# jeremy-collins/sd-video-gen

Hardware: AMD Instinct MI355X
Metric: generated frames/sec at 50 DDIM denoise steps, 512x512 (higher is better)
Workload: dtype fp16; 1 GPU; configs[2]: 1_16_kitti_L1_64 F=64, 64x64 latents -> 512x512 VAE passes, 50-step DDIM; --denoise --denoise_start_step 0, guidance_scale 0; SD-v1.4 UNet at 64x64 latents, VAE enc/dec at 512x512; clips_per_gpu=56, streams_per_gpu=2, pred_frames=1, global_clips=56, parallelism=clip-sharded dp1, weights=seeded random init (SD v1.4 architecture, 1_16_kitti_L1_64)

## Files before the change

sd-video-gen_amd/csrc/ff_fused.hip:

```cpp
#include "igemm_epi.h"
#include <vector>

namespace SDNS {

namespace {

constexpr int FC = 320;
constexpr int FH = 1280;
constexpr int F_SLAB = 16384;
#ifndef FF_DEPTH
#define FF_DEPTH 4
#endif
constexpr int F_DEPTH = FF_DEPTH;
constexpr int F_KS = FC / 32;
constexpr int F_NCH = FH / 64;
constexpr int F_SPC = 5 + 3;

struct FfArgs {
  const h16* X; int ldx;
  const h16* W1; const float* b1; const float* s1;
  const float* rs; const float* rm;
  const h16* W2p; const float* b2;
  const h16* residual; int ldr;
  h16* out; int ldo;
  int M;
};

constexpr int P_RING = 7;
constexpr int P_OFF_S1 = P_RING * F_SLAB;
constexpr int P_OFF_EX = P_OFF_S1 + 2 * 2 * FH * 4;
constexpr int P_LDS = P_OFF_EX + 8 * 2 * 64 * 16;

#ifdef FF_STAMP
#define FSTAMP(v) do { __builtin_amdgcn_sched_barrier(0); asm volatile("s_memtime %0\n\ts_waitcnt lgkmcnt(0)" : "=s"(v) :: "memory"); __builtin_amdgcn_sched_barrier(0); } while (0)
#else
#define FSTAMP(v) do { } while (0)
#endif

__global__ void __launch_bounds__(512, 2) ff_pair_kernel(const FfArgs a, unsigned long long* stamps) {
  extern __shared__ __attribute__((aligned(16))) char smem[];
  const int tid = threadIdx.x, lane = tid & 63, wid = tid >> 6;
  const int wave_u = __builtin_amdgcn_readfirstlane(wid);
  const int pair_u = wave_u >> 1, half_u = wave_u & 1;
  const int l15 = lane & 15, lq = lane >> 4;
  const int m0 = blockIdx.x * 128;
  const unsigned lds0 = (unsigned)(uintptr_t)((__attribute__((address_space(3))) char*)smem);
  constexpr unsigned INVALID = 0x80000000u;

  const uint64_t p1 = (uint64_t)a.W1, p2 = (uint64_t)a.W2p;
  const v4i srd1 = {(int)(unsigned)p1, (int)((p1 >> 32) & 0xffff), (int)(2u * FH * FC * 2u), 0x00020000};
  const v4i srd2 = {(int)(unsigned)p2, (int)((p2 >> 32) & 0xffff), (int)((unsigned)FC * FH * 2u), 0x00020000};

  const int prow = lane >> 3;
  auto dma_slab = [&](int q, int slot) {
    const int c = q >> 3, s = q & 7;
    const unsigned dst = lds0 + slot * F_SLAB;
#pragma unroll
    for (int i = 0; i < 2; ++i) {
      const int blk = i * 8 + wave_u;
      const int row = blk * 8 + prow;
      const int ch = (lane & 7) ^ (row & 7);
      if (s < 5) {
        const unsigned voff = (unsigned)((128 * c + row) * FC + ch * 8) * 2u;
        dma16(srd1, voff, s * 128, dst + blk * 1024);
      } else {
        const int rr = 64 * (s - 5) + (row & 63);
        const int cperm = 32 * (rr >> 5) + 8 * ((rr & 15) >> 2) + 4 * ((rr >> 4) & 1) + (rr & 3);
        const int r = (row >> 6) * 160 + cperm;
        const unsigned voff = rr < 160 ? (unsigned)(r * FH + ch * 8) * 2u : INVALID;
        dma16(srd2, voff, c * 128, dst + blk * 1024);
      }
    }
  };
  constexpr int NQ = F_NCH * F_SPC;
#pragma unroll
  for (int q = 0; q < F_DEPTH; ++q) dma_slab(q, q);

  {
    float* ss = (float*)(smem + P_OFF_S1);
    for (int i = tid; i < 2 * FH; i += 512) { ss[i] = a.s1[i]; ss[2 * FH + i] = a.b1[i]; }
    asm volatile("s_waitcnt lgkmcnt(0)" ::: "memory");
  }
  int mrow[2]; bool m_ok[2];
  h16x8 xf[2][F_KS];
#pragma unroll
  for (int rt = 0; rt < 2; ++rt) {
    mrow[rt] = m0 + pair_u * 32 + rt * 16 + l15;
    m_ok[rt] = mrow[rt] < a.M;
#pragma unroll
    for (int ks = 0; ks < F_KS; ++ks) {
      uint4 v = make_uint4(0, 0, 0, 0);
      if (m_ok[rt]) v = *(const uint4*)(a.X + (int64_t)mrow[rt] * a.ldx + ks * 32 + lq * 8);
      xf[rt][ks] = *(h16x8*)&v;
    }
  }
  float rs[2], rm[2];
#pragma unroll
  for (int rt = 0; rt < 2; ++rt) {
    if (a.rs) {
      rs[rt] = m_ok[rt] ? a.rs[mrow[rt]] : 0.f; rm[rt] = m_ok[rt] ? a.rm[mrow[rt]] : 0.f;
    } else {
      float sum = 0.f;
#pragma unroll
      for (int ks = 0; ks < F_KS; ++ks)
#pragma unroll
        for (int j = 0; j < 8; ++j) sum += (float)xf[rt][ks][j];
      sum += __shfl_xor(sum, 16); sum += __shfl_xor(sum, 32);
      const float mean = sum * (1.f / FC);
      float sq = 0.f;
#pragma unroll
      for (int ks = 0; ks < F_KS; ++ks)
#pragma unroll
        for (int j = 0; j < 8; ++j) { const float dlt = (float)xf[rt][ks][j] - mean; sq += dlt * dlt; }
      sq += __shfl_xor(sq, 16); sq += __shfl_xor(sq, 32);
      rs[rt] = m_ok[rt] ? rsqrtf(sq * (1.f / FC) + 1e-5f) : 0.f;
      rm[rt] = rs[rt] * mean;
    }
  }

  f32x4 acc2[2][10];
#pragma unroll
  for (int rt = 0; rt < 2; ++rt)
#pragma unroll
    for (int t = 0; t < 10; ++t) acc2[rt][t] = f32x4{0.f, 0.f, 0.f, 0.f};

  int fsw[2];
#pragma unroll
  for (int kk = 0; kk < 2; ++kk) fsw[kk] = (half_u * 64 + l15) * 128 + (((kk * 4 + lq) ^ (l15 & 7)) << 4);
  const float* const sS1 = (const float*)(smem + P_OFF_S1);
  const float* const sB1 = sS1 + 2 * FH;
  char* const ex_own = smem + P_OFF_EX + ((wave_u * 2) * 64 + lane) * 16;
  const char* const ex_other = smem + P_OFF_EX + (((wave_u ^ 1) * 2) * 64 + lane) * 16;

  int q = 0, slot = 0, slot_in = F_DEPTH;
  unsigned long long t_wait = 0, t_bar = 0, t_dma = 0, t_g1 = 0, t_gelu = 0, t_g2 = 0, t_all0 = 0, t_all1 = 0, t_epi = 0;
  auto step_sync = [&]() {
    unsigned long long u0 = 0, u1 = 0, u2 = 0;
    FSTAMP(u0);
    if (q + F_DEPTH - 1 < NQ) asm volatile("s_waitcnt vmcnt(6)" ::: "memory");
    else wait_vm((NQ - 1 - q) * 2);
    FSTAMP(u1);
    bar();
    FSTAMP(u2);
    t_wait += u1 - u0; t_bar += u2 - u1;
  };
  auto step_dma = [&]() {
    unsigned long long u2 = 0, u3 = 0;
    FSTAMP(u2);
    if (q + F_DEPTH < NQ) dma_slab(q + F_DEPTH, slot_in);
    FSTAMP(u3);
    t_dma += u3 - u2;
    slot_in = slot_in + 1 == P_RING ? 0 : slot_in + 1;
  };
  auto step_end = [&]() { ++q; slot = slot + 1 == P_RING ? 0 : slot + 1; };
#ifndef FF_STAGGER
#define FF_STAGGER 1
#endif
  const bool late = FF_STAGGER && wave_u >= 4;

  FSTAMP(t_all0);
  for (int c = 0; c < F_NCH; ++c) {
    f32x4 acc1[2][4];
#pragma unroll
    for (int rt = 0; rt < 2; ++rt)
#pragma unroll
      for (int t = 0; t < 4; ++t) acc1[rt][t] = f32x4{0.f, 0.f, 0.f, 0.f};
    h16x8 wpend[4];
    auto rd1 = [&](const char* sl, int kk, h16x8 (&wf)[4]) {
#pragma unroll
      for (int t = 0; t < 4; ++t) wf[t] = *(const h16x8*)(sl + t * 2048 + fsw[kk]);
    };
    auto mm1 = [&](int ks, const h16x8 (&wf)[4]) {
#pragma unroll
      for (int t = 0; t < 4; ++t)
#pragma unroll
        for (int rt = 0; rt < 2; ++rt) acc1[rt][t] = MFMA_16x16x32(wf[t], xf[rt][ks], acc1[rt][t]);
    };
#pragma unroll
    for (int s = 0; s < 5; ++s) {
      step_sync();
      unsigned long long v0 = 0, v1 = 0;
      FSTAMP(v0);
      const char* sl = smem + slot * F_SLAB;
      if (late && s > 0) mm1((s - 1) * 2 + 1, wpend);
      step_dma();
      {
        h16x8 wf[4];
        rd1(sl, 0, wf);
        mm1(s * 2, wf);
      }
      rd1(sl, 1, wpend);
      if (!late || s == 4) mm1(s * 2 + 1, wpend);
#ifdef FF_STAMP
#pragma unroll
      for (int rt = 0; rt < 2; ++rt)
#pragma unroll
        for (int t = 0; t < 4; ++t) asm volatile("" : "+v"(acc1[rt][t]));
#endif
      FSTAMP(v1);
      t_g1 += v1 - v0;
      step_end();
    }
    unsigned long long w0 = 0, w1 = 0;
    FSTAMP(w0);
    h16x8 pown[2];
#pragma unroll
    for (int rt = 0; rt < 2; ++rt) {
#pragma unroll
      for (int pr = 0; pr < 2; ++pr) {
        const int n = 128 * c + 64 * half_u + 32 * pr + 4 * lq;
        const f32x4 sh = *(const f32x4*)(sS1 + n), sg = *(const f32x4*)(sS1 + n + 16);
        const f32x4 bh = *(const f32x4*)(sB1 + n), bg = *(const f32x4*)(sB1 + n + 16);
        const f32x4 h = acc1[rt][2 * pr] * rs[rt] - sh * rm[rt] + bh;
        const f32x4 gt = acc1[rt][2 * pr + 1] * rs[rt] - sg * rm[rt] + bg;
        const f32x4 pv = h * gelu_erf4(gt);
#pragma unroll
        for (int e = 0; e < 4; ++e) pown[rt][pr * 4 + e] = (h16)pv[e];
      }
      *(h16x8*)(ex_own + rt * 1024) = pown[rt];
    }
    asm volatile("s_waitcnt lgkmcnt(0)" ::: "memory");
    FSTAMP(w1);
    t_gelu += w1 - w0;
    h16x8 pf[2][2];
    auto rd2 = [&](const char* sl, int kk, h16x8 (&wf)[4]) {
#pragma unroll
      for (int t = 0; t < 4; ++t) wf[t] = *(const h16x8*)(sl + t * 2048 + fsw[kk]);
    };
    auto mm2 = [&](int s, int kk, const h16x8 (&wf)[4]) {
#pragma unroll
      for (int t = 0; t < 4; ++t) {
        if (s * 4 + t < 10) {
#pragma unroll
          for (int rt = 0; rt < 2; ++rt) acc2[rt][s * 4 + t] = MFMA_16x16x32(wf[t], pf[rt][kk], acc2[rt][s * 4 + t]);
        }
      }
    };
#pragma unroll
    for (int s = 0; s < 3; ++s) {
      step_sync();
      unsigned long long v0 = 0, v1 = 0;
      FSTAMP(v0);
      if (s == 0) {
#pragma unroll
        for (int rt = 0; rt < 2; ++rt) {
          const h16x8 po = *(const h16x8*)(ex_other + rt * 1024);
          pf[rt][0] = half_u ? po : pown[rt];
          pf[rt][1] = half_u ? pown[rt] : po;
        }
      }
      const char* sl = smem + slot * F_SLAB;
      if (late && s > 0) mm2(s - 1, 1, wpend);
      step_dma();
      {
        h16x8 wf[4];
        rd2(sl, 0, wf);
        mm2(s, 0, wf);
      }
      rd2(sl, 1, wpend);
      if (!late || s == 2) mm2(s, 1, wpend);
#ifdef FF_STAMP
#pragma unroll
      for (int rt = 0; rt < 2; ++rt)
#pragma unroll
        for (int t = 0; t < 4; ++t) if (s * 4 + t < 10) asm volatile("" : "+v"(acc2[rt][s * 4 + t]));
#endif
      FSTAMP(v1);
      t_g2 += v1 - v0;
      step_end();
    }
  }
  FSTAMP(t_all1);

#pragma unroll
  for (int rt = 0; rt < 2; ++rt) {
    if (!m_ok[rt]) continue;
    const int m = mrow[rt];
#pragma unroll
    for (int p = 0; p < 5; ++p) {
      const int n = half_u * 160 + 32 * p + 8 * lq;
      f32x4 v0 = acc2[rt][2 * p] + *(const f32x4*)(a.b2 + n);
      f32x4 v1 = acc2[rt][2 * p + 1] + *(const f32x4*)(a.b2 + n + 4);
      if (a.residual) {
        const h16x8 r = *(const h16x8*)(a.residual + (int64_t)m * a.ldr + n);
#pragma unroll
        for (int e = 0; e < 4; ++e) { v0[e] += (float)r[e]; v1[e] += (float)r[4 + e]; }
      }
      h16x8 w;
      const h16x4 w0 = to_h16x4(v0), w1 = to_h16x4(v1);
#pragma unroll
      for (int e = 0; e < 4; ++e) { w[e] = w0[e]; w[4 + e] = w1[e]; }
      *(h16x8*)(a.out + (int64_t)m * a.ldo + n) = w;
    }
  }
#ifdef FF_STAMP
  FSTAMP(t_epi);
  if (stamps && lane == 0) {
    unsigned long long* o = stamps + ((size_t)blockIdx.x * 8 + wid) * 8;
    o[0] = t_wait; o[1] = t_bar; o[2] = t_dma; o[3] = t_g1; o[4] = t_gelu; o[5] = t_g2; o[6] = t_all1 - t_all0; o[7] = t_epi - t_all1;
  }
#endif
}

__global__ void pack_ff2_perm_kernel(const float* __restrict__ w, h16* __restrict__ out, int N, int K) {
  const int64_t total = (int64_t)N * K;
  for (int64_t idx = (int64_t)blockIdx.x * blockDim.x + threadIdx.x; idx < total; idx += (int64_t)gridDim.x * blockDim.x) {
    const int n = (int)(idx / K), k = (int)(idx - (int64_t)n * K);
    const int b = k >> 5, p = k & 31, lq = p >> 3, j = p & 7;
    out[idx] = (h16)w[(int64_t)n * K + 32 * b + 16 * (j >> 2) + 4 * lq + (j & 3)];
  }
}

}

void ff_fused_init_device() {
  HIP_OK(hipFuncSetAttribute((const void*)ff_pair_kernel, hipFuncAttributeMaxDynamicSharedMemorySize, P_LDS));
}

bool ff_fused_supported(int C, int M) {
  return C == FC && M >= 128 * 192;
}

void pack_ff2_perm(const float* w, h16* out, int N, int K, hipStream_t s) {
  const int64_t total = (int64_t)N * K;
  hipLaunchKernelGGL(pack_ff2_perm_kernel, dim3((unsigned)std::min<int64_t>((total + 255) / 256, 4096)), dim3(256), 0, s, w, out, N, K);
  check_launch("pack_ff2_perm");
}

void ff_fused(svg_ctx* ctx, const h16* X, int ldx, const h16* W1, const float* b1, const float* s1,
              const h16* W2p, const float* b2, const h16* residual, int ldr, h16* out, int ldo, int M, hipStream_t s) {
  SVG_CHECK(ldx % 8 == 0 && ldr % 8 == 0 && ldo % 8 == 0 && (int64_t)M * ldx < (1LL << 31), "ff_fused: strides / size unsupported");
  if (!SVG_LAUNCHING(ctx)) return;
  char tag[64];
  snprintf(tag, sizeof(tag), "ff_fused_M%d_C%d", M, FC);
  ProfScope ps(ctx, PK_GEMM, s, 2.0 * M * (double)FC * (2 * FH) + 2.0 * M * (double)FH * FC,
               2.0 * ((double)M * FC * 3 + 3.0 * FC * FH), tag);
  FfArgs a{X, ldx, W1, b1, s1, nullptr, nullptr, W2p, b2, residual, ldr, out, ldo, M};
  unsigned long long* stamps = nullptr;
#ifdef FF_STAMP
  const size_t n_st = (size_t)cdiv(M, 128) * 64;
  HIP_OK(hipMalloc(&stamps, n_st * sizeof(unsigned long long)));
  HIP_OK(hipMemsetAsync(stamps, 0, n_st * sizeof(unsigned long long), s));
#endif
  hipLaunchKernelGGL(ff_pair_kernel, dim3(cdiv(M, 128)), dim3(512), P_LDS, s, a, stamps);
  check_launch("ff_fused");
#ifdef FF_STAMP
  {
    HIP_OK(hipStreamSynchronize(s));
    std::vector<unsigned long long> h(n_st);
    HIP_OK(hipMemcpy(h.data(), stamps, n_st * sizeof(unsigned long long), hipMemcpyDeviceToHost));
    HIP_OK(hipFree(stamps));
    double sum[8] = {0};
    for (size_t w = 0; w < n_st / 8; ++w) for (int k = 0; k < 8; ++k) sum[k] += (double)h[w * 8 + k];
    const double nw = (double)(n_st / 8);
    fprintf(stderr, "[ff stamps] M %d: per wave (cycles, 160 slab steps): ring wait %.0f | barrier %.0f | DMA issue %.0f | GEMM1 slabs (100 x: 8 reads + 16 MFMA) %.0f | "
            "LN-fold + GEGLU + swap write (20 x) %.0f | GEMM2 slabs (60 x: reads + up to 16 MFMA) %.0f || main loop %.0f, epilogue %.0f; matrix time of the loop = 2400 MFMA x 16 = 38400\n",
            M, sum[0] / nw, sum[1] / nw, sum[2] / nw, sum[3] / nw, sum[4] / nw, sum[5] / nw, sum[6] / nw, sum[7] / nw);
  }
#endif
}

}
```

sd-video-gen_amd/csrc/xattn_fused.hip:

```cpp
#include "igemm_epi.h"
#include <cstdlib>

namespace SDNS {

namespace {

constexpr int XC = 320, XH = 8, XD = 40, XDP = 48;
constexpr int XQ = XH * XDP;
constexpr int X_SLAB = 16384;
constexpr int X_RING = 8, X_DEPTH = 4;
constexpr int X_KS = XC / 32;
constexpr int X_P0 = 15, X_P1 = 15, X_P2 = 2 * XH, X_P3 = 18;
constexpr int X_OFF_C = X_RING * X_SLAB;
constexpr int X_LDS = X_OFF_C + (2 * XQ + XC) * 4;
constexpr int X_HEAD_ELEMS = 128 * 64;

struct XaArgs {
  const h16* X; int ldx;
  const h16* R; int ldr;
  const h16* Wp; const float* bp;
  const float* rs; const float* rm;
  const h16* Wq; const float* sq; const float* bq;
  const h16* Kp; const h16* Vp;
  const h16* Wo; const float* bo;
  h16* out; int ldo;
  int M, rows_per_sample, L;
  float scale_log2e;
};

__device__ __forceinline__ h16x8 cat8(h16x4 a, h16x4 b) { return __builtin_shufflevector(a, b, 0, 1, 2, 3, 4, 5, 6, 7); }

template <bool CHAIN>
__global__ void __launch_bounds__(512, 2) xattn_fused_kernel(const XaArgs a) {
  constexpr int Q0 = CHAIN ? X_P0 : 0;
  constexpr int X_NQ = Q0 + X_P1 + X_P2 + X_P3;
  extern __shared__ __attribute__((aligned(16))) char smem[];
  const int tid = threadIdx.x, lane = tid & 63, wid = tid >> 6;
  const int wave_u = __builtin_amdgcn_readfirstlane(wid);
  const int l15 = lane & 15, lq = lane >> 4;
  const int m0 = blockIdx.x * 128;
  const int sample = m0 / a.rows_per_sample;
  const unsigned lds0 = (unsigned)(uintptr_t)((__attribute__((address_space(3))) char*)smem);
  constexpr unsigned INVALID = 0x80000000u;

  const uint64_t pq = (uint64_t)a.Wq, po = (uint64_t)a.Wo, pp = (uint64_t)a.Wp;
  const v4i srdp = {(int)(unsigned)pp, (int)((pp >> 32) & 0xffff), (int)((unsigned)XC * XC * 2u), 0x00020000};
  const uint64_t pk = (uint64_t)(a.Kp + (int64_t)sample * XH * X_HEAD_ELEMS), pv = (uint64_t)(a.Vp + (int64_t)sample * XH * X_HEAD_ELEMS);
  const v4i srdq = {(int)(unsigned)pq, (int)((pq >> 32) & 0xffff), (int)((unsigned)XQ * XC * 2u), 0x00020000};
  const v4i srdo = {(int)(unsigned)po, (int)((po >> 32) & 0xffff), (int)((unsigned)XC * XQ * 2u), 0x00020000};
  const v4i srdk = {(int)(unsigned)pk, (int)((pk >> 32) & 0xffff), (int)((unsigned)XH * X_HEAD_ELEMS * 2u), 0x00020000};
  const v4i srdv = {(int)(unsigned)pv, (int)((pv >> 32) & 0xffff), (int)((unsigned)XH * X_HEAD_ELEMS * 2u), 0x00020000};

  const int prow = lane >> 3;
  auto dma_slab = [&](int qq) {
    const unsigned dst = lds0 + (qq & (X_RING - 1)) * X_SLAB;
    const int q = qq - Q0;
#pragma unroll
    for (int i = 0; i < 2; ++i) {
      const int blk = i * 8 + wave_u;
      const int row = blk * 8 + prow;
      const int ch = (lane & 7) ^ (row & 7);
      if (CHAIN && q < 0) {
        const int ks = qq / 3, rb = qq - 3 * ks;
        const int r = rb * 128 + row;
        dma16(srdp, r < XC ? (unsigned)((r * XC + ch * 8) * 2) : INVALID, ks * 128, dst + blk * 1024);
      } else if (q < X_P1) {
        const int ks = q / 3, rb = q - 3 * ks;
        dma16(srdq, (unsigned)(((rb * 128 + row) * XC + ch * 8) * 2), ks * 128, dst + blk * 1024);
      } else if (q < X_P1 + X_P2) {
        const int j = q - X_P1, h = j >> 1;
        const unsigned voff = (unsigned)((row * 64 + ch * 8) * 2);
        if (j & 1) dma16(srdv, voff, h * X_HEAD_ELEMS * 2, dst + blk * 1024);
        else dma16(srdk, voff, h * X_HEAD_ELEMS * 2, dst + blk * 1024);
      } else {
        const int j = q - X_P1 - X_P2, ks = j / 3, rb = j - 3 * ks;
        const int x = rb * 128 + row;
        const int r = CHAIN ? x : 32 * (x >> 5) + 8 * ((x & 15) >> 2) + 4 * ((x >> 4) & 1) + (x & 3);
        dma16(srdo, x < XC ? (unsigned)((r * XQ + ch * 8) * 2) : INVALID, ks * 128, dst + blk * 1024);
      }
    }
  };
#pragma unroll
  for (int q = 0; q < X_DEPTH; ++q) dma_slab(q);

  float* const sSq = (float*)(smem + X_OFF_C);
  float* const sBq = sSq + XQ;
  float* const sBo = sBq + XQ;
  for (int i = tid; i < XQ; i += 512) { sSq[i] = a.sq[i]; sBq[i] = a.bq[i]; }
  for (int i = tid; i < XC; i += 512) sBo[i] = a.bo[i];
  asm volatile("s_waitcnt lgkmcnt(0)" ::: "memory");

  const int m = m0 + wave_u * 16 + l15;
  const bool m_ok = m < a.M;
  h16x8 xf[X_KS];
#pragma unroll
  for (int ks = 0; ks < X_KS; ++ks) {
    uint4 v = make_uint4(0, 0, 0, 0);
    if (m_ok) v = *(const uint4*)(a.X + (int64_t)m * a.ldx + ks * 32 + lq * 8);
    xf[ks] = *(h16x8*)&v;
  }
  int fsw[2];
#pragma unroll
  for (int kk = 0; kk < 2; ++kk) fsw[kk] = l15 * 128 + (((kk * 4 + lq) ^ (l15 & 7)) << 4);

  int q = 0;
  auto step_begin = [&]() {
    if (q + X_DEPTH - 1 < X_NQ) asm volatile("s_waitcnt vmcnt(6)" ::: "memory");
    else wait_vm((X_NQ - 1 - q) * 2);
    bar();
    if (q + X_DEPTH < X_NQ) dma_slab(q + X_DEPTH);
  };
  const h16x4 zero4 = {(h16)0.f, (h16)0.f, (h16)0.f, (h16)0.f};

  h16x4 hb[XC / 16];
  float rs, rm;
  if (CHAIN) {
    f32x4 acc0[XC / 16];
#pragma unroll
    for (int t = 0; t < XC / 16; ++t) acc0[t] = f32x4{0.f, 0.f, 0.f, 0.f};
#pragma unroll
    for (int ks = 0; ks < 5; ++ks)
#pragma unroll
      for (int rb = 0; rb < 3; ++rb) {
        step_begin();
        const char* sl = smem + (q & (X_RING - 1)) * X_SLAB;
#pragma unroll
        for (int kk = 0; kk < 2; ++kk)
#pragma unroll
          for (int t = 0; t < 8; ++t)
            if (rb * 8 + t < XC / 16) {
              const h16x8 wf = *(const h16x8*)(sl + t * 2048 + fsw[kk]);
              acc0[rb * 8 + t] = MFMA_16x16x32(wf, xf[ks * 2 + kk], acc0[rb * 8 + t]);
            }
        ++q;
      }
    float sum = 0.f;
#pragma unroll
    for (int t = 0; t < XC / 16; ++t) {
      const int n = t * 16 + lq * 4;
      f32x4 v = acc0[t] + *(const f32x4*)(a.bp + n);
      if (m_ok) {
        const h16x4 r = *(const h16x4*)(a.R + (int64_t)m * a.ldr + n);
        v[0] += (float)r[0]; v[1] += (float)r[1]; v[2] += (float)r[2]; v[3] += (float)r[3];
      }
      hb[t] = to_h16x4(v);
#pragma unroll
      for (int e = 0; e < 4; ++e) sum += (float)hb[t][e];
    }
    sum += __shfl_xor(sum, 16); sum += __shfl_xor(sum, 32);
    const float mean = sum * (1.f / XC);
    float sq = 0.f;
#pragma unroll
    for (int t = 0; t < XC / 16; ++t)
#pragma unroll
      for (int e = 0; e < 4; ++e) { const float dlt = (float)hb[t][e] - mean; sq += dlt * dlt; }
    sq += __shfl_xor(sq, 16); sq += __shfl_xor(sq, 32);
    rs = m_ok ? rsqrtf(sq * (1.f / XC) + 1e-5f) : 0.f;
    rm = rs * mean;
  } else if (a.rs) {
    rs = m_ok ? a.rs[m] : 0.f; rm = m_ok ? a.rm[m] : 0.f;
  } else {
    float sum = 0.f;
#pragma unroll
    for (int ks = 0; ks < X_KS; ++ks)
#pragma unroll
      for (int j = 0; j < 8; ++j) sum += (float)xf[ks][j];
    sum += __shfl_xor(sum, 16); sum += __shfl_xor(sum, 32);
    const float mean = sum * (1.f / XC);
    float sq = 0.f;
#pragma unroll
    for (int ks = 0; ks < X_KS; ++ks)
#pragma unroll
      for (int j = 0; j < 8; ++j) { const float dlt = (float)xf[ks][j] - mean; sq += dlt * dlt; }
    sq += __shfl_xor(sq, 16); sq += __shfl_xor(sq, 32);
    rs = m_ok ? rsqrtf(sq * (1.f / XC) + 1e-5f) : 0.f;
    rm = rs * mean;
  }

  h16x4 qb[3 * XH];
  {
    f32x4 accq[3 * XH];
#pragma unroll
    for (int t = 0; t < 3 * XH; ++t) accq[t] = f32x4{0.f, 0.f, 0.f, 0.f};
#pragma unroll
    for (int ks = 0; ks < 5; ++ks)
#pragma unroll
      for (int rb = 0; rb < 3; ++rb) {
        step_begin();
        const char* sl = smem + (q & (X_RING - 1)) * X_SLAB;
#pragma unroll
        for (int kk = 0; kk < 2; ++kk) {
          h16x8 wf[8];
#pragma unroll
          for (int t = 0; t < 8; ++t) wf[t] = *(const h16x8*)(sl + t * 2048 + fsw[kk]);
#pragma unroll
          for (int t = 0; t < 8; ++t)
            accq[rb * 8 + t] = MFMA_16x16x32(wf[t], CHAIN ? cat8(hb[2 * (ks * 2 + kk)], hb[2 * (ks * 2 + kk) + 1]) : xf[ks * 2 + kk], accq[rb * 8 + t]);
        }
        ++q;
      }
#pragma unroll
    for (int t = 0; t < 3 * XH; ++t) {
      const int n = t * 16 + lq * 4;
      const f32x4 sv = *(const f32x4*)(sSq + n), bv = *(const f32x4*)(sBq + n);
      qb[t] = to_h16x4((accq[t] * rs - sv * rm + bv) * a.scale_log2e);
    }
  }

  h16x4 ob[3 * XH];
#pragma unroll
  for (int h = 0; h < XH; ++h) {
    step_begin();
    f32x4 sacc[5];
    {
      const char* sl = smem + (q & (X_RING - 1)) * X_SLAB;
#pragma unroll
      for (int t = 0; t < 5; ++t) sacc[t] = f32x4{0.f, 0.f, 0.f, 0.f};
#pragma unroll
      for (int kk = 0; kk < 2; ++kk) {
        const h16x8 bop = cat8(qb[3 * h + 2 * kk], kk == 0 ? qb[3 * h + 1] : zero4);
#pragma unroll
        for (int t = 0; t < 5; ++t) {
          const h16x8 wf = *(const h16x8*)(sl + t * 2048 + fsw[kk]);
          sacc[t] = MFMA_16x16x32(wf, bop, sacc[t]);
        }
      }
      ++q;
    }
    float mx = -INFINITY;
#pragma unroll
    for (int t = 0; t < 5; ++t)
#pragma unroll
      for (int e = 0; e < 4; ++e) {
        if (16 * t + 4 * lq + e >= a.L) sacc[t][e] = -INFINITY;
        mx = fmaxf(mx, sacc[t][e]);
      }
    mx = fmaxf(mx, __shfl_xor(mx, 16)); mx = fmaxf(mx, __shfl_xor(mx, 32));
    h16x4 pb[5];
    float sum = 0.f;
#pragma unroll
    for (int t = 0; t < 5; ++t) {
      f32x4 p;
#pragma unroll
      for (int e = 0; e < 4; ++e) p[e] = __builtin_amdgcn_exp2f(sacc[t][e] - mx);
      pb[t] = to_h16x4(p);
#pragma unroll
      for (int e = 0; e < 4; ++e) sum += (float)pb[t][e];
    }
    sum += __shfl_xor(sum, 16); sum += __shfl_xor(sum, 32);
    step_begin();
    {
      const char* sl = smem + (q & (X_RING - 1)) * X_SLAB;
      f32x4 oacc[3];
#pragma unroll
      for (int dt = 0; dt < 3; ++dt) oacc[dt] = f32x4{0.f, 0.f, 0.f, 0.f};
#pragma unroll
      for (int s = 0; s < 3; ++s) {
        const int c = s >> 1, kk = s & 1;
        const h16x8 bop = cat8(pb[2 * s], s < 2 ? pb[2 * s + 1] : zero4);
#pragma unroll
        for (int dt = 0; dt < 3; ++dt) {
          const h16x8 wf = *(const h16x8*)(sl + (c * 3 + dt) * 2048 + fsw[kk]);
          oacc[dt] = MFMA_16x16x32(wf, bop, oacc[dt]);
        }
      }
      ++q;
      const float inv = __builtin_amdgcn_rcpf(sum);
#pragma unroll
      for (int dt = 0; dt < 3; ++dt) ob[3 * h + dt] = to_h16x4(oacc[dt] * inv);
    }
  }

  f32x4 acco[XC / 16];
#pragma unroll
  for (int t = 0; t < XC / 16; ++t) acco[t] = f32x4{0.f, 0.f, 0.f, 0.f};
#pragma unroll
  for (int ks = 0; ks < 6; ++ks)
#pragma unroll
    for (int rb = 0; rb < 3; ++rb) {
      step_begin();
      const char* sl = smem + (q & (X_RING - 1)) * X_SLAB;
#pragma unroll
      for (int kk = 0; kk < 2; ++kk) {
        const int s = 2 * ks + kk;
        const h16x8 bop = cat8(ob[2 * s], ob[2 * s + 1]);
#pragma unroll
        for (int t = 0; t < 8; ++t)
          if (rb * 8 + t < XC / 16) {
            const h16x8 wf = *(const h16x8*)(sl + t * 2048 + fsw[kk]);
            acco[rb * 8 + t] = MFMA_16x16x32(wf, bop, acco[rb * 8 + t]);
          }
      }
      ++q;
    }

  if (m_ok) {
    if constexpr (CHAIN) {
#pragma unroll
      for (int t = 0; t < XC / 16; ++t) {
        const int n = t * 16 + lq * 4;
        f32x4 v = acco[t] + *(const f32x4*)(sBo + n);
        const h16x4 r = hb[t];
        v[0] += (float)r[0]; v[1] += (float)r[1]; v[2] += (float)r[2]; v[3] += (float)r[3];
        *(h16x4*)(a.out + (int64_t)m * a.ldo + n) = to_h16x4(v);
      }
    } else {
#pragma unroll
      for (int p = 0; p < XC / 32; ++p) {
        const int n = 32 * p + 8 * lq;
        f32x4 v0 = acco[2 * p] + *(const f32x4*)(sBo + n), v1 = acco[2 * p + 1] + *(const f32x4*)(sBo + n + 4);
        const h16x8 r = *(const h16x8*)(a.X + (int64_t)m * a.ldx + n);
#pragma unroll
        for (int e = 0; e < 4; ++e) { v0[e] += (float)r[e]; v1[e] += (float)r[4 + e]; }
        *(h16x8*)(a.out + (int64_t)m * a.ldo + n) = cat8(to_h16x4(v0), to_h16x4(v1));
      }
    }
  }
}

__device__ __forceinline__ int perm32(int p) {
  const int b = p >> 5, r = p & 31, lq = r >> 3, j = r & 7;
  return 32 * b + 16 * (j >> 2) + 4 * lq + (j & 3);
}

__global__ void xattn_pack_q_kernel(const float* __restrict__ w, const float* __restrict__ gamma, const float* __restrict__ beta,
                                    h16* __restrict__ Wq, float* __restrict__ bq, int perm) {
  const int r = blockIdx.x;
  const int h = r / XDP, j = r - h * XDP;
  float acc = 0.f;
  for (int p = threadIdx.x; p < XC; p += blockDim.x) {
    const int k = perm ? perm32(p) : p;
    const float v = j < XD ? w[(int64_t)(h * XD + j) * XC + k] : 0.f;
    Wq[(int64_t)r * XC + p] = (h16)(v * gamma[k]);
    acc += v * beta[k];
  }
  __shared__ float red[256];
  red[threadIdx.x] = acc;
  __syncthreads();
  for (int s = blockDim.x / 2; s > 0; s >>= 1) { if ((int)threadIdx.x < s) red[threadIdx.x] += red[threadIdx.x + s]; __syncthreads(); }
  if (threadIdx.x == 0) bq[r] = red[0];
}

__global__ void xattn_pack_o_kernel(const float* __restrict__ w, h16* __restrict__ Wo) {
  const int n = blockIdx.x;
  for (int p = threadIdx.x; p < XQ; p += blockDim.x) {
    const int c = perm32(p), h = c / XDP, dd = c - h * XDP;
    Wo[(int64_t)n * XQ + p] = (h16)(dd < XD ? w[(int64_t)n * XC + h * XD + dd] : 0.f);
  }
}

__global__ void xattn_pack_kv_kernel(const h16* __restrict__ K, int ldk, int64_t k_bs, const h16* __restrict__ Vt, int ldv, int64_t v_bs,
                                     h16* __restrict__ Kp, h16* __restrict__ Vp, int L) {
  const int n = blockIdx.y, h = blockIdx.x;
  h16* kp = Kp + ((int64_t)n * XH + h) * X_HEAD_ELEMS;
  h16* vp = Vp + ((int64_t)n * XH + h) * X_HEAD_ELEMS;
  for (int i = threadIdx.x; i < X_HEAD_ELEMS; i += blockDim.x) {
    const int row = i >> 6, p = i & 63, c = perm32(p);
    kp[i] = (row < L && c < XD) ? K[(int64_t)n * k_bs + (int64_t)row * ldk + h * XD + c] : (h16)0.f;
    const int chunk = row / XDP, dd = row - chunk * XDP, key = 64 * chunk + c;
    vp[i] = (chunk < 2 && dd < XD && key < L) ? Vt[(int64_t)n * v_bs + (int64_t)(h * XD + dd) * ldv + key] : (h16)0.f;
  }
}

}

void xattn_fused_init_device() {
  HIP_OK(hipFuncSetAttribute((const void*)xattn_fused_kernel<false>, hipFuncAttributeMaxDynamicSharedMemorySize, X_LDS));
  HIP_OK(hipFuncSetAttribute((const void*)xattn_fused_kernel<true>, hipFuncAttributeMaxDynamicSharedMemorySize, X_LDS));
}

bool xattn_fused_supported(int C, int heads, int M, int rows_per_sample, int L) {
  if (svg_env_i64("SVG_XATTN_FUSED", 1) == 0) return false;
  return C == XC && heads == XH && L > 0 && L <= 80 && rows_per_sample % 128 == 0 && M % rows_per_sample == 0 && M >= 128 * 192;
}
bool xattn_chain_enabled() {
  return svg_env_i64("SVG_XATTN_FUSED", 1) >= 2;
}

int64_t xattn_kv_pack_elems(int N) { return (int64_t)N * XH * X_HEAD_ELEMS; }

void xattn_pack_q(const float* w, const float* gamma, const float* beta, h16* Wq, float* sq, float* bq, int perm, hipStream_t s) {
  hipLaunchKernelGGL(xattn_pack_q_kernel, dim3(XQ), dim3(256), 0, s, w, gamma, beta, Wq, bq, perm);
  check_launch("xattn_pack_q");
  rowsum_h16(Wq, sq, XQ, XC, s);
}

void xattn_pack_o(const float* w, h16* Wo, hipStream_t s) {
  hipLaunchKernelGGL(xattn_pack_o_kernel, dim3(XC), dim3(128), 0, s, w, Wo);
  check_launch("xattn_pack_o");
}

void xattn_pack_kv(const h16* K, int ldk, int64_t k_bs, const h16* Vt, int ldv, int64_t v_bs, h16* Kp, h16* Vp, int N, int L, hipStream_t s) {
  hipLaunchKernelGGL(xattn_pack_kv_kernel, dim3(XH, N), dim3(256), 0, s, K, ldk, k_bs, Vt, ldv, v_bs, Kp, Vp, L);
  check_launch("xattn_pack_kv");
}

void xattn_fused(svg_ctx* ctx, const h16* X, int ldx, const h16* R, int ldr, const h16* Wp, const float* bp, const float* rs, const float* rm,
                 const h16* Wq, const float* sq, const float* bq, const h16* Kp, const h16* Vp, const h16* Wo, const float* bo, h16* out, int ldo,
                 int M, int rows_per_sample, int L, hipStream_t s) {
  SVG_CHECK(ldx % 8 == 0 && ldo % 8 == 0 && (int64_t)M * ldx < (1LL << 31) && (!Wp || (R && ldr % 4 == 0)), "xattn_fused: strides / size unsupported");
  if (!SVG_LAUNCHING(ctx)) return;
  char tag[64];
  snprintf(tag, sizeof(tag), "xattn_%s_M%d_C%d_L%d", Wp ? "chain" : "fused", M, XC, L);
  ProfScope ps(ctx, PK_ATTN, s, 2.0 * M * (double)XC * XC * (Wp ? 3 : 2) + 4.0 * M * (double)L * XC, 2.0 * ((double)M * XC * (Wp ? 3 : 2) + (Wp ? 3.0 : 2.0) * XC * XC), tag);
  XaArgs a{X, ldx, R, ldr, Wp, bp, rs, rm, Wq, sq, bq, Kp, Vp, Wo, bo, out, ldo, M, rows_per_sample, L, 1.4426950408889634f / sqrtf((float)XD)};
  if (Wp) hipLaunchKernelGGL(xattn_fused_kernel<true>, dim3(cdiv(M, 128)), dim3(512), X_LDS, s, a);
  else hipLaunchKernelGGL(xattn_fused_kernel<false>, dim3(cdiv(M, 128)), dim3(512), X_LDS, s, a);
  check_launch("xattn_fused");
}

}
```

Baseline: 18.69 frames/s.

## Interleave weight-slab DMA instructions between MFMAs in FF and cross-attn kernels

Instead of issuing both per-wave buffer-to-LDS DMA instructions for the next weight slab right after the barrier, the FF and cross-attention kernels now place them at chosen positions inside the MFMA sequence. Scheduling barriers pin them there. The FF address math is restructured so the per-lane offset is loop-invariant and the slab-dependent part moves into the scalar offset, which cuts VALU work per DMA. The FF epilogue also hoists the bias and residual loads before the output loop. The aim is to hide DMA issue cost behind matrix-core work, with the risk that the pinned scheduling barriers constrain the compiler and stall MFMA chains.

```diff
diff --git a/sd-video-gen_amd/csrc/ff_fused.hip b/sd-video-gen_amd/csrc/ff_fused.hip
--- a/sd-video-gen_amd/csrc/ff_fused.hip
+++ b/sd-video-gen_amd/csrc/ff_fused.hip
@@ -26,6 +26,12 @@
   int M;
 };
 
+#ifndef FF_DMA_M
+#define FF_DMA_M 2
+#endif
+constexpr int F_DMA_M = FF_DMA_M;
+static_assert(F_DMA_M >= 0 && F_DMA_M <= 2, "a slab is two DMA instructions per wave");
+__host__ __device__ constexpr int ff_dma_at(int i, int n) { return i * (n / 2) + n / 4 - 1; }
 constexpr int P_RING = 7;
 constexpr int P_OFF_S1 = P_RING * F_SLAB;
 constexpr int P_OFF_EX = P_OFF_S1 + 2 * 2 * FH * 4;
@@ -52,26 +58,26 @@
   const v4i srd2 = {(int)(unsigned)p2, (int)((p2 >> 32) & 0xffff), (int)((unsigned)FC * FH * 2u), 0x00020000};
 
   const int prow = lane >> 3;
-  auto dma_slab = [&](int q, int slot) {
+  auto dma_part = [&](int q, int slot, int i0, int i1) {
     const int c = q >> 3, s = q & 7;
     const unsigned dst = lds0 + slot * F_SLAB;
 #pragma unroll
-    for (int i = 0; i < 2; ++i) {
+    for (int i = i0; i < i1; ++i) {
       const int blk = i * 8 + wave_u;
-      const int row = blk * 8 + prow;
-      const int ch = (lane & 7) ^ (row & 7);
+      const int r0 = wave_u * 8 + prow;
+      const int ch = (lane & 7) ^ (r0 & 7);
       if (s < 5) {
-        const unsigned voff = (unsigned)((128 * c + row) * FC + ch * 8) * 2u;
-        dma16(srd1, voff, s * 128, dst + blk * 1024);
+        const unsigned voff = (unsigned)(r0 * FC + ch * 8) * 2u;
+        dma16(srd1, voff, c * (128 * FC * 2) + i * (64 * FC * 2) + s * 128, dst + blk * 1024);
       } else {
-        const int rr = 64 * (s - 5) + (row & 63);
-        const int cperm = 32 * (rr >> 5) + 8 * ((rr & 15) >> 2) + 4 * ((rr >> 4) & 1) + (rr & 3);
-        const int r = (row >> 6) * 160 + cperm;
-        const unsigned voff = rr < 160 ? (unsigned)(r * FH + ch * 8) * 2u : INVALID;
-        dma16(srd2, voff, c * 128, dst + blk * 1024);
+        const int rr = 64 * (s - 5) + r0;
+        const int cperm0 = 32 * (r0 >> 5) + 8 * ((r0 & 15) >> 2) + 4 * ((r0 >> 4) & 1) + (r0 & 3);
+        const unsigned voff = rr < 160 ? (unsigned)(cperm0 * FH + ch * 8) * 2u : INVALID;
+        dma16(srd2, voff, i * (160 * FH * 2) + (s - 5) * (64 * FH * 2) + c * 128, dst + blk * 1024);
       }
     }
   };
+  auto dma_slab = [&](int q, int slot) { dma_part(q, slot, 0, 2); };
   constexpr int NQ = F_NCH * F_SPC;
 #pragma unroll
   for (int q = 0; q < F_DEPTH; ++q) dma_slab(q, q);
@@ -147,11 +153,21 @@
   auto step_dma = [&]() {
     unsigned long long u2 = 0, u3 = 0;
     FSTAMP(u2);
-    if (q + F_DEPTH < NQ) dma_slab(q + F_DEPTH, slot_in);
+    if (F_DMA_M < 2 && q + F_DEPTH < NQ) dma_part(q + F_DEPTH, slot_in, 0, 2 - F_DMA_M);
     FSTAMP(u3);
     t_dma += u3 - u2;
     slot_in = slot_in + 1 == P_RING ? 0 : slot_in + 1;
   };
+  int slot_ld = 0;
+  auto ride = [&](bool on, int idx, int n) {
+#pragma unroll
+    for (int i = 2 - F_DMA_M; i < 2; ++i)
+      if (idx == ff_dma_at(i, n)) {
+        __builtin_amdgcn_sched_barrier(0);
+        if (on) dma_part(q + F_DEPTH, slot_ld, i, i + 1);
+        __builtin_amdgcn_sched_barrier(0);
+      }
+  };
   auto step_end = [&]() { ++q; slot = slot + 1 == P_RING ? 0 : slot + 1; };
 #ifndef FF_STAGGER
 #define FF_STAGGER 1
@@ -170,11 +186,14 @@
 #pragma unroll
       for (int t = 0; t < 4; ++t) wf[t] = *(const h16x8*)(sl + t * 2048 + fsw[kk]);
     };
-    auto mm1 = [&](int ks, const h16x8 (&wf)[4]) {
+    auto mm1 = [&](int ks, const h16x8 (&wf)[4], bool dma, int nr) {
 #pragma unroll
       for (int t = 0; t < 4; ++t)
 #pragma unroll
-        for (int rt = 0; rt < 2; ++rt) acc1[rt][t] = MFMA_16x16x32(wf[t], xf[rt][ks], acc1[rt][t]);
+        for (int rt = 0; rt < 2; ++rt) {
+          acc1[rt][t] = MFMA_16x16x32(wf[t], xf[rt][ks], acc1[rt][t]);
+          ride(dma, t * 2 + rt, nr);
+        }
     };
 #pragma unroll
     for (int s = 0; s < 5; ++s) {
@@ -182,15 +201,17 @@
       unsigned long long v0 = 0, v1 = 0;
       FSTAMP(v0);
       const char* sl = smem + slot * F_SLAB;
-      if (late && s > 0) mm1((s - 1) * 2 + 1, wpend);
+      const bool more = q + F_DEPTH < NQ, carried = late && s > 0;
+      slot_ld = slot_in;
+      if (carried) mm1((s - 1) * 2 + 1, wpend, more, 8);
       step_dma();
       {
         h16x8 wf[4];
         rd1(sl, 0, wf);
-        mm1(s * 2, wf);
+        mm1(s * 2, wf, more && late, s == 0 ? 8 : 0);
       }
       rd1(sl, 1, wpend);
-      if (!late || s == 4) mm1(s * 2 + 1, wpend);
+      if (!late || s == 4) mm1(s * 2 + 1, wpend, more && !late, 8);
 #ifdef FF_STAMP
 #pragma unroll
       for (int rt = 0; rt < 2; ++rt)
@@ -227,12 +248,15 @@
 #pragma unroll
       for (int t = 0; t < 4; ++t) wf[t] = *(const h16x8*)(sl + t * 2048 + fsw[kk]);
     };
-    auto mm2 = [&](int s, int kk, const h16x8 (&wf)[4]) {
+    auto mm2 = [&](int s, int kk, const h16x8 (&wf)[4], bool dma, bool carrier) {
 #pragma unroll
       for (int t = 0; t < 4; ++t) {
         if (s * 4 + t < 10) {
 #pragma unroll
-          for (int rt = 0; rt < 2; ++rt) acc2[rt][s * 4 + t] = MFMA_16x16x32(wf[t], pf[rt][kk], acc2[rt][s * 4 + t]);
+          for (int rt = 0; rt < 2; ++rt) {
+            acc2[rt][s * 4 + t] = MFMA_16x16x32(wf[t], pf[rt][kk], acc2[rt][s * 4 + t]);
+            ride(dma, t * 2 + rt, carrier ? (s < 2 ? 8 : 4) : 0);
+          }
         }
       }
     };
@@ -250,15 +274,17 @@
         }
       }
       const char* sl = smem + slot * F_SLAB;
-      if (late && s > 0) mm2(s - 1, 1, wpend);
+      const bool more = q + F_DEPTH < NQ, carried = late && s > 0;
+      slot_ld = slot_in;
+      if (carried) mm2(s - 1, 1, wpend, more, true);
       step_dma();
       {
         h16x8 wf[4];
         rd2(sl, 0, wf);
-        mm2(s, 0, wf);
+        mm2(s, 0, wf, more && late, s == 0);
       }
       rd2(sl, 1, wpend);
-      if (!late || s == 2) mm2(s, 1, wpend);
+      if (!late || s == 2) mm2(s, 1, wpend, more && !late, true);
 #ifdef FF_STAMP
 #pragma unroll
       for (int rt = 0; rt < 2; ++rt)
@@ -272,6 +298,20 @@
   }
   FSTAMP(t_all1);
 
+  f32x4 bb[5][2];
+  h16x8 rr[2][5];
+#pragma unroll
+  for (int p = 0; p < 5; ++p) {
+    const int n = half_u * 160 + 32 * p + 8 * lq;
+    bb[p][0] = *(const f32x4*)(a.b2 + n); bb[p][1] = *(const f32x4*)(a.b2 + n + 4);
+  }
+  if (a.residual) {
+#pragma unroll
+    for (int rt = 0; rt < 2; ++rt)
+#pragma unroll
+      for (int p = 0; p < 5; ++p)
+        if (m_ok[rt]) rr[rt][p] = *(const h16x8*)(a.residual + (int64_t)mrow[rt] * a.ldr + half_u * 160 + 32 * p + 8 * lq);
+  }
 #pragma unroll
   for (int rt = 0; rt < 2; ++rt) {
     if (!m_ok[rt]) continue;
@@ -279,10 +319,10 @@
 #pragma unroll
     for (int p = 0; p < 5; ++p) {
       const int n = half_u * 160 + 32 * p + 8 * lq;
-      f32x4 v0 = acc2[rt][2 * p] + *(const f32x4*)(a.b2 + n);
-      f32x4 v1 = acc2[rt][2 * p + 1] + *(const f32x4*)(a.b2 + n + 4);
+      f32x4 v0 = acc2[rt][2 * p] + bb[p][0];
+      f32x4 v1 = acc2[rt][2 * p + 1] + bb[p][1];
       if (a.residual) {
-        const h16x8 r = *(const h16x8*)(a.residual + (int64_t)m * a.ldr + n);
+        const h16x8 r = rr[rt][p];
 #pragma unroll
         for (int e = 0; e < 4; ++e) { v0[e] += (float)r[e]; v1[e] += (float)r[4 + e]; }
       }
diff --git a/sd-video-gen_amd/csrc/xattn_fused.hip b/sd-video-gen_amd/csrc/xattn_fused.hip
--- a/sd-video-gen_amd/csrc/xattn_fused.hip
+++ b/sd-video-gen_amd/csrc/xattn_fused.hip
@@ -28,6 +28,13 @@
   float scale_log2e;
 };
 
+#ifndef XA_DMA_M
+#define XA_DMA_M 2
+#endif
+constexpr int XA_M = XA_DMA_M;
+static_assert(XA_M >= 0 && XA_M <= 2, "a slab is two DMA instructions per wave");
+__host__ __device__ constexpr int xa_dma_at(int i, int n) { return n / 2 + (i ? 3 * n / 8 : n / 8); }
+
 __device__ __forceinline__ h16x8 cat8(h16x4 a, h16x4 b) { return __builtin_shufflevector(a, b, 0, 1, 2, 3, 4, 5, 6, 7); }
 
 template <bool CHAIN>
@@ -52,11 +59,11 @@
   const v4i srdv = {(int)(unsigned)pv, (int)((pv >> 32) & 0xffff), (int)((unsigned)XH * X_HEAD_ELEMS * 2u), 0x00020000};
 
   const int prow = lane >> 3;
-  auto dma_slab = [&](int qq) {
+  auto dma_part = [&](int qq, int i0, int i1) {
     const unsigned dst = lds0 + (qq & (X_RING - 1)) * X_SLAB;
     const int q = qq - Q0;
 #pragma unroll
-    for (int i = 0; i < 2; ++i) {
+    for (int i = i0; i < i1; ++i) {
       const int blk = i * 8 + wave_u;
       const int row = blk * 8 + prow;
       const int ch = (lane & 7) ^ (row & 7);
@@ -81,7 +88,7 @@
     }
   };
 #pragma unroll
-  for (int q = 0; q < X_DEPTH; ++q) dma_slab(q);
+  for (int q = 0; q < X_DEPTH; ++q) dma_part(q, 0, 2);
 
   float* const sSq = (float*)(smem + X_OFF_C);
   float* const sBq = sSq + XQ;
@@ -108,7 +115,16 @@
     if (q + X_DEPTH - 1 < X_NQ) asm volatile("s_waitcnt vmcnt(6)" ::: "memory");
     else wait_vm((X_NQ - 1 - q) * 2);
     bar();
-    if (q + X_DEPTH < X_NQ) dma_slab(q + X_DEPTH);
+    if (XA_M < 2 && q + X_DEPTH < X_NQ) dma_part(q + X_DEPTH, 0, 2 - XA_M);
+  };
+  auto ride = [&](int idx, int n) {
+#pragma unroll
+    for (int i = 2 - XA_M; i < 2; ++i)
+      if (idx == xa_dma_at(i, n) && q + X_DEPTH < X_NQ) {
+        __builtin_amdgcn_sched_barrier(0);
+        dma_part(q + X_DEPTH, i, i + 1);
+        __builtin_amdgcn_sched_barrier(0);
+      }
   };
   const h16x4 zero4 = {(h16)0.f, (h16)0.f, (h16)0.f, (h16)0.f};
 
@@ -131,6 +147,7 @@
             if (rb * 8 + t < XC / 16) {
               const h16x8 wf = *(const h16x8*)(sl + t * 2048 + fsw[kk]);
               acc0[rb * 8 + t] = MFMA_16x16x32(wf, xf[ks * 2 + kk], acc0[rb * 8 + t]);
+              ride(kk * (rb < 2 ? 8 : 4) + t, rb < 2 ? 16 : 8);
             }
         ++q;
       }
@@ -194,8 +211,10 @@
 #pragma unroll
           for (int t = 0; t < 8; ++t) wf[t] = *(const h16x8*)(sl + t * 2048 + fsw[kk]);
 #pragma unroll
-          for (int t = 0; t < 8; ++t)
+          for (int t = 0; t < 8; ++t) {
             accq[rb * 8 + t] = MFMA_16x16x32(wf[t], CHAIN ? cat8(hb[2 * (ks * 2 + kk)], hb[2 * (ks * 2 + kk) + 1]) : xf[ks * 2 + kk], accq[rb * 8 + t]);
+            ride(kk * 8 + t, 16);
+          }
         }
         ++q;
       }
@@ -223,6 +242,7 @@
         for (int t = 0; t < 5; ++t) {
           const h16x8 wf = *(const h16x8*)(sl + t * 2048 + fsw[kk]);
           sacc[t] = MFMA_16x16x32(wf, bop, sacc[t]);
+          ride(kk * 5 + t, 10);
         }
       }
       ++q;
@@ -262,6 +282,7 @@
         for (int dt = 0; dt < 3; ++dt) {
           const h16x8 wf = *(const h16x8*)(sl + (c * 3 + dt) * 2048 + fsw[kk]);
           oacc[dt] = MFMA_16x16x32(wf, bop, oacc[dt]);
+          ride(s * 3 + dt, 9);
         }
       }
       ++q;
@@ -289,6 +310,7 @@
           if (rb * 8 + t < XC / 16) {
             const h16x8 wf = *(const h16x8*)(sl + t * 2048 + fsw[kk]);
             acco[rb * 8 + t] = MFMA_16x16x32(wf, bop, acco[rb * 8 + t]);
+            ride(kk * (rb < 2 ? 8 : 4) + t, rb < 2 ? 16 : 8);
           }
       }
       ++q;
```

After: 18.76 frames/s, median of 6. Within noise of the previous version (+0.4%).
